# bfloat16/latent-diffusion-speech

Hardware: AMD Instinct MI355X
Metric: mel_frames_per_sec (higher is better)
Workload: dtype f32; 1 GPU; configs[1]: batch=16x512-frame utterances per GPU, 50-step dpm-solver, unet1d denoiser, 80-ch mel; pipeline=sampler, utterances_per_gpu=16, frames=512, nfe=50, method=dpm-solver, parallelism=batch-shard x1

## Files before the change

latent-diffusion-speech_amd/csrc/host_stub_hip.cpp:

```cpp
#include <hip/hip_runtime_api.h>

#include <stdlib.h>
#include <string.h>

extern "C" {
hipError_t hipMalloc(void** p, size_t n) {
    *p = malloc(n ? n : 1);
    return *p ? hipSuccess : hipErrorOutOfMemory;
}
hipError_t hipFree(void* p) {
    free(p);
    return hipSuccess;
}
hipError_t hipMemcpy(void* d, const void* s, size_t n, hipMemcpyKind) {
    memcpy(d, s, n);
    return hipSuccess;
}
hipError_t hipMemcpyAsync(void* d, const void* s, size_t n, hipMemcpyKind, hipStream_t) {
    memcpy(d, s, n);
    return hipSuccess;
}
hipError_t hipMemsetAsync(void* d, int v, size_t n, hipStream_t) {
    memset(d, v, n);
    return hipSuccess;
}
hipError_t hipMemcpy2DAsync(void* d, size_t dpitch, const void* s_, size_t spitch, size_t width, size_t height, hipMemcpyKind, hipStream_t) {
    for (size_t r = 0; r < height; ++r) memcpy((char*)d + r * dpitch, (const char*)s_ + r * spitch, width);
    return hipSuccess;
}
hipError_t hipMemsetD32Async(hipDeviceptr_t d, int v, size_t count, hipStream_t) {
    for (size_t i = 0; i < count; ++i) memcpy((char*)d + 4 * i, &v, 4);
    return hipSuccess;
}
hipError_t hipStreamSynchronize(hipStream_t) { return hipSuccess; }
hipError_t hipGetDevice(int* d) {
    *d = 0;
    return hipSuccess;
}
hipError_t hipGetLastError(void) { return hipSuccess; }
hipError_t hipDeviceGetAttribute(int*, hipDeviceAttribute_t, int) { return hipErrorNotSupported; }
const char* hipGetErrorString(hipError_t) { return "host stub"; }
hipError_t hipFuncSetAttribute(const void*, hipFuncAttribute, int) { return hipSuccess; }
hipError_t hipLaunchKernel(const void*, dim3, dim3, void**, size_t, hipStream_t) { return hipErrorNotSupported; }
hipError_t hipExtLaunchKernel(const void*, dim3, dim3, void**, size_t, hipStream_t, hipEvent_t, hipEvent_t, int) { return hipErrorNotSupported; }
hipError_t hipEventCreate(hipEvent_t*) { return hipErrorNotSupported; }
hipError_t hipEventDestroy(hipEvent_t) { return hipSuccess; }
hipError_t hipEventRecord(hipEvent_t, hipStream_t) { return hipErrorNotSupported; }
hipError_t hipEventSynchronize(hipEvent_t) { return hipErrorNotSupported; }
hipError_t hipEventElapsedTime(float*, hipEvent_t, hipEvent_t) { return hipErrorNotSupported; }
void** __hipRegisterFatBinary(const void*) {
    static void* handle = nullptr;
    return &handle;
}
void __hipRegisterFunction(void**, const void*, char*, const char*, unsigned int, void*, void*, void*, void*, int*) {}
void __hipRegisterVar(void**, void*, char*, const char*, int, size_t, int, int) {}
void __hipUnregisterFatBinary(void**) {}
hipError_t __hipPushCallConfiguration(dim3, dim3, size_t, hipStream_t) { return hipSuccess; }
hipError_t __hipPopCallConfiguration(dim3*, dim3*, size_t*, hipStream_t*) { return hipErrorNotSupported; }
}
```

latent-diffusion-speech_amd/csrc/kernels.h:

```cpp
#pragma once
#include <hip/hip_runtime.h>
#include <stddef.h>
#include <stdint.h>

#include <atomic>
#include <string>

namespace lds {

enum { ACT_NONE = 0, ACT_LRELU = 2 };
enum { EPI_NONE = 0, EPI_GEGLU = 1, EPI_TANH = 2, EPI_GELU = 3, EPI_SWISH = 4, EPI_GLU = 5 };

struct ConvArgs {
    const float* x1; const float* x2;
    int C1, C2;
    int Tsrc;
    int Tin;
    long long xb1, xb2;
    const float* w;
    int Mp, Co, Ci, KT, stride, dil, pad, ups;
    int act_in; float slope;
    const float* bias;
    const float* bias_bc;
    const float* res;
// ... 151 lines not shown
hipError_t launch_w2v_lnpart(const float* x, float2* part, const int* nlen, int B, int C, int T, hipStream_t s);

constexpr int kW2vbertRelStride = 80;
hipError_t launch_w2vbert_fbank(const float* audio, const int* slen, long long L, int Nmax, int Rmax, const double* basis, const float* filtT, int n_mels,
                                int stride, float mel_floor, float* logspec, double2* stat, float* out, int B, hipStream_t s);
hipError_t launch_w2vbert_feats_k4p(const float* feats, float* out, float2* part, const int* vlen, int B, int C, int T, hipStream_t s);
hipError_t launch_w2vbert_relpos(const float* qk, const float* E, float* relp, const int* qlen, int B, int C, int T, int heads, int NR, hipStream_t s);
hipError_t launch_attention_k4p_rel(const float* qk, const float* vt, const float* relp, float* out, int B, int C, int T, int heads, const int* qlens,
                                    const int* klens, int left, int right, hipStream_t s);
hipError_t launch_w2vbert_dwconv(const float* x, const float* wp, const float* gamma, const float* beta, float eps, float* out, const int* vlen,
                                 const int* nlen, int B, int C, int T, int K, hipStream_t s);

enum { IN_PLAIN = 0, IN_SILU = 1, IN_SINUSOID = 2 };
hipError_t launch_small_linear(const float* W, const float* bias, const float* in, int in_stride, int in_mode,
                               const float* freqs, float* out, int out_stride, int out_silu, int M, int K, int B, hipStream_t s);

enum {
    EW_X0 = 1,
    EW_AXPBY = 2,
    EW_DPM2 = 3,
    EW_UNIPC_PRED = 4,
    EW_UNIPC_CORR = 5,
    EW_UNIPC_CORR1 = 6,
    EW_DDPM = 7,
    EW_DDIM = 8,
    EW_PLMS_PRED = 9,
    EW_LIN4 = 10,
    EW_COPY = 11
};
hipError_t launch_ew(int op, float* out, const float* a, const float* b, const float* c, const float* d,
                     float c0, float c1, float c2, float c3, float c4, long long n, hipStream_t s);
hipError_t launch_dpm_step(float* x, const float* eps, float* m0, const float* m1, float sigma, float alpha, int second, float c4, float c5, float c6,
                           float c7, long long n, hipStream_t s);
hipError_t launch_fill(float* p, float v, long long n, hipStream_t s);
hipError_t launch_touch_lines(const float* p, long long bytes, hipStream_t s);
struct FloatList64 { float f[64]; };
hipError_t launch_set_list(float* dst, const float* host, int n, hipStream_t s);
hipError_t launch_transpose(const float* in, float* out, int B, int R, int C, float scale, hipStream_t s);
hipError_t launch_gather_rows(const float* table, const int64_t* idx, int idx_off, float* out, int B, int C,
                              int nrows, hipStream_t s);
hipError_t launch_resample_frames(const float* in, float* out, int B, int Tin, int Tout, int C, float step, hipStream_t s);
hipError_t launch_resample_nearest(const float* in, float* out, int B, int C, int Tin, int Tout, hipStream_t s);


bool prof_attach_events(hipEvent_t* start, hipEvent_t* stop);
int set_error(int code, const char* fmt, ...);

struct ProfScope {
    bool on;
    hipStream_t s;
    int idx = -1;
    bool attached = false;
    ProfScope(hipStream_t st, const char* name, double flops, double bytes, bool attachable = false);
    ~ProfScope();
    void rename(const std::string& n);
};

inline hipError_t ensure_max_dynamic_lds(const void* kern, std::atomic<unsigned long long>& done) {
    int dev = 0;
    hipError_t e = hipGetDevice(&dev);
    if (e != hipSuccess) return e;
    const unsigned long long bit = 1ull << (dev & 63);
    if (done.load(std::memory_order_acquire) & bit) return hipSuccess;
    e = hipFuncSetAttribute(kern, hipFuncAttributeMaxDynamicSharedMemorySize, 160 * 1024);
    if (e == hipSuccess) done.fetch_or(bit, std::memory_order_release);
    return e;
// ... 4 lines not shown
```

latent-diffusion-speech_amd/csrc/misc.hip:

```cpp
#include "kernels.h"
#include "../../include/lds.h"

#include <math.h>

namespace lds {

template <int BT>
__global__ void __launch_bounds__(256) small_linear_kernel(const float* __restrict__ W, const float* __restrict__ bias,
                                                           const float* __restrict__ in, int in_stride, int in_mode,
                                                           const float* __restrict__ freqs, float* __restrict__ out,
                                                           int out_stride, int out_silu, int M, int K, int B) {
    const int lane = threadIdx.x & 63;
    const int m = blockIdx.x * 4 + (threadIdx.x >> 6);
    if (m >= M) return;
    const float* wr = W + (long long)m * K;
    for (int b0 = 0; b0 < B; b0 += BT) {
        float acc[BT];
#pragma unroll
        for (int i = 0; i < BT; ++i) acc[i] = 0.f;
        for (int k = lane * 4; k < K; k += 256) {
            const float4 w4 = *reinterpret_cast<const float4*>(wr + k);
            const float wv[4] = {w4.x, w4.y, w4.z, w4.w};
#pragma unroll
            for (int i = 0; i < BT; ++i) {
// ... 68 lines not shown
            default: r = a[i]; break;
        }
        out[i] = r;
    }
}

hipError_t launch_ew(int op, float* out, const float* a, const float* b, const float* c, const float* d, float c0, float c1,
                     float c2, float c3, float c4, long long n, hipStream_t s) {
    long long blocks = (n + 255) / 256;
    if (blocks > 4096) blocks = 4096;
    ProfScope ps(s, "ew", 0.0, 4.0 * 3.0 * (double)n);
    hipLaunchKernelGGL(ew_kernel, dim3((unsigned)blocks), dim3(256), 0, s, op, out, a, b, c, d, c0, c1, c2, c3, c4, n);
    return hipGetLastError();
}

__global__ void __launch_bounds__(256) dpm_step_kernel(float* __restrict__ x, const float* __restrict__ eps, float* __restrict__ m0, const float* __restrict__ m1,
                                                       float sigma, float alpha, int second, float c4, float c5, float c6, float c7, long long n) {
    for (long long i = (long long)blockIdx.x * 256 + threadIdx.x; i < n; i += (long long)gridDim.x * 256) {
        const float xi = x[i];
        const float bi = (xi - sigma * eps[i]) / alpha;
        m0[i] = bi;
        x[i] = second ? c4 * xi - c5 * bi - c6 * (c7 * (bi - m1[i])) : c4 * xi - c5 * bi;
    }
}
hipError_t launch_dpm_step(float* x, const float* eps, float* m0, const float* m1, float sigma, float alpha, int second, float c4, float c5, float c6,
                           float c7, long long n, hipStream_t s) {
    long long blocks = (n + 255) / 256;
    if (blocks > 4096) blocks = 4096;
    ProfScope ps(s, "ew", 0.0, 4.0 * (second ? 5.0 : 4.0) * (double)n);
    hipLaunchKernelGGL(dpm_step_kernel, dim3((unsigned)blocks), dim3(256), 0, s, x, eps, m0, m1, sigma, alpha, second, c4, c5, c6, c7, n);
    return hipGetLastError();
}

__global__ void __launch_bounds__(256) fill_kernel(float* p, float v, long long n) {
    for (long long i = (long long)blockIdx.x * 256 + threadIdx.x; i < n; i += (long long)gridDim.x * 256) p[i] = v;
}
__global__ void __launch_bounds__(256) touch_lines_kernel(const float* p, long long n_lines, float* sink) {
    const long long i = (long long)blockIdx.x * 256 + threadIdx.x;
    float v = 0.f;
    if (i < n_lines) v = p[i * 16];
    if (v == 1.2345678e-30f && sink) sink[0] = v;
}
hipError_t launch_touch_lines(const float* p, long long bytes, hipStream_t s) {
    const long long n_lines = bytes / 64;
    if (n_lines <= 0) return hipSuccess;
    hipLaunchKernelGGL(touch_lines_kernel, dim3((unsigned)((n_lines + 255) / 256)), dim3(256), 0, s, p, n_lines, (float*)nullptr);
    return hipGetLastError();
}

hipError_t launch_fill(float* p, float v, long long n, hipStream_t s) {
    long long blocks = (n + 255) / 256;
    if (blocks > 4096) blocks = 4096;
    ProfScope ps(s, "fill", 0.0, 4.0 * (double)n);
    hipLaunchKernelGGL(fill_kernel, dim3((unsigned)blocks), dim3(256), 0, s, p, v, n);
    return hipGetLastError();
}

__global__ void __launch_bounds__(64) set_list_kernel(float* __restrict__ dst, FloatList64 v, int n) {
    if ((int)threadIdx.x < n) dst[threadIdx.x] = v.f[threadIdx.x];
}
hipError_t launch_set_list(float* dst, const float* host, int n, hipStream_t s) {
    if (n < 0 || n > 64) return hipErrorInvalidValue;
    FloatList64 v;
    for (int i = 0; i < 64; ++i) v.f[i] = i < n ? host[i] : 0.f;
    hipLaunchKernelGGL(set_list_kernel, dim3(1), dim3(64), 0, s, dst, v, n);
    return hipGetLastError();
// ... 171 lines not shown
```

latent-diffusion-speech_amd/csrc/model.hip:

```cpp
#include "../../include/lds.h"
#include "../../include/lds_test.h"
#include "k4p.h"
#include "k8b3.h"
#include "kernels.h"

#include <math.h>
#include <stdarg.h>
#include <stdio.h>
#include <stdlib.h>
#include <string.h>

#include <algorithm>
#include <atomic>
#include <map>
#include <mutex>
#include <string>
#include <vector>

using namespace lds;

static thread_local char g_err[512] = "";
static int fail(int code, const char* fmt, ...) {
    va_list ap;
    va_start(ap, fmt);
// ... 647 lines not shown
    return LDS_OK;
}

static int dconv_any(int mode, const ConvW& W, const float* x1, int C1, const float* x2, int C2, int Tsrc, const DOpt& o, float* out, int B, hipStream_t st) {
    return mode ? run_dconv_bf3(W, x1, C1, x2, C2, Tsrc, o, out, B, st, 0, mode - 1) : run_dconv(W, x1, C1, x2, C2, Tsrc, o, out, B, st);
}
static hipError_t gn_any(int mode, const float* x1, const float* x2, int C1, int C2, int T, int groups, float eps, const float* gamma, const float* beta,
                         const float* ss, int ss_stride, int ss_off, int silu, const float2* gp1, const float2* gp2, float* y, int B, hipStream_t s, int lvl = 0) {
    return mode ? launch_gn_stream_bf3(x1, x2, C1, C2, T, groups, eps, gamma, beta, ss, ss_stride, ss_off, silu, gp1, gp2, y, B, s, mode - 1, tl_lens, lvl)
                : launch_gn_stream(x1, x2, C1, C2, T, groups, eps, gamma, beta, ss, ss_stride, ss_off, silu, gp1, gp2, y, B, s, tl_lens, lvl);
}
static hipError_t to_act_any(int mode, const float* in, float* out, int B, int C, int T, int Ctot, int c_off, hipStream_t s) {
    return mode ? launch_to_k8b3(in, out, B, C, T, Ctot, c_off, s, mode - 1, tl_lens) : launch_to_k4p(in, out, B, C, T, Ctot, c_off, s, tl_lens);
}

struct ResnetW {
    int cin = 0, cout = 0;
    float *g1 = nullptr, *b1 = nullptr, *g2 = nullptr, *b2 = nullptr;
    ConvW conv1, conv2, sc;
    float* bias_pair = nullptr;
    bool has_sc = false;
    int temb_off = 0;
};
struct TfmW {
    int C = 0;
    float *gn_g = nullptr, *gn_b = nullptr;
    float *qkv_c1[2] = {nullptr, nullptr}, *qkv_c2[2] = {nullptr, nullptr}, *ff1_c1 = nullptr, *ff1_c2 = nullptr;
    ConvW proj_in, qkv[2], o[2], ff1, ff2_out;
    ConvW proj_in_g; float *pi_cg = nullptr, *pi_c2 = nullptr; bool fold = false;
};
struct DownBlk { std::vector<ResnetW> res; std::vector<TfmW> att; bool has_down = false; ConvW down; int ch = 0; };
struct UpBlk { std::vector<ResnetW> res; std::vector<TfmW> att; std::vector<int> skip_ch; bool has_up = false; ConvW up; int ch = 0; };

struct lds_unet {
    lds_unet_cfg cfg;
    Owner own;
    int M = 0, H = 0, G = 8, heads = 8, temb = 0, tproj_dim = 0;
    ConvW conv_in, conv_out;
    ConvW conv_in_x, conv_in_c;
    float *gno_g = nullptr, *gno_b = nullptr;
    float* freqs = nullptr;
    float *t_w1 = nullptr, *t_b1 = nullptr, *t_w2 = nullptr, *t_b2 = nullptr;
    float *tp_w = nullptr, *tp_b = nullptr;
    int tp_M = 0;
    std::vector<DownBlk> down;
    ResnetW mid_r0, mid_r1;
    TfmW mid_t;
    std::vector<UpBlk> up;
    int max_ci = 0;
    int gemm_mode = LDS_GEMM_F32;
    bool split_packed[2] = {false, false};
    int latency_mode = 0;
    std::atomic<int> in_calls{0};
};
struct UnetCallScope {
    lds_unet* u;
    explicit UnetCallScope(lds_unet* u_) : u(u_) { u->in_calls.fetch_add(1, std::memory_order_acq_rel); }
    ~UnetCallScope() { u->in_calls.fetch_sub(1, std::memory_order_acq_rel); }
};

static float* up_vec(Owner& o, const float* p, int64_t n) {
    if (!p) return nullptr;
    return o.upload(std::vector<float>(p, p + n));
}

static bool load_resnet(lds_unet* u, Tensors& T, const std::string& p, int cin, int cout, std::vector<float>& tpw,
                        std::vector<float>& tpb, ResnetW& r) {
    Owner& o = u->own;
    r.cin = cin; r.cout = cout;
    r.g1 = up_vec(o, T.get(p + "norm1.weight", cin), cin);
    r.b1 = up_vec(o, T.get(p + "norm1.bias", cin), cin);
    r.g2 = up_vec(o, T.get(p + "norm2.weight", cout), cout);
    r.b2 = up_vec(o, T.get(p + "norm2.bias", cout), cout);
    const float* w1 = T.get(p + "conv1.weight", (int64_t)cout * cin * 3);
    const float* c1b = T.get(p + "conv1.bias", cout);
    const float* w2 = T.get(p + "conv2.weight", (int64_t)cout * cout * 3);
    const float* c2b = T.get(p + "conv2.bias", cout);
    const float* tw = T.get(p + "time_emb_proj.weight", (int64_t)2 * cout * u->temb);
    const float* tb = T.get(p + "time_emb_proj.bias", 2 * cout);
    if (!r.g1 || !r.b1 || !r.g2 || !r.b2 || !w1 || !c1b || !w2 || !c2b || !tw || !tb) return false;
    if (!pack_conv(o, w1, c1b, cout, cin, 3, r.conv1)) return false;
    if (!pack_conv(o, w2, c2b, cout, cout, 3, r.conv2)) return false;
    r.has_sc = cin != cout;
    if (r.has_sc) {
        const float* ws = T.get(p + "conv_shortcut.weight", (int64_t)cout * cin);
// ... 173 lines not shown
        for (int j = 0; j < L + 1 && ok; ++j) {
            const int sk = skip_ch.back();
            skip_ch.pop_back();
            const int hin = j == 0 ? prev : cout;
            b.skip_ch.push_back(sk);
            ResnetW r;
            ok = load_resnet(u, T, p + "resnets." + std::to_string(j) + ".", hin + sk, cout, tpw, tpb, r);
            b.res.push_back(r);
            if (i != 0 && ok) {
                TfmW t;
                ok = load_tfm(u, T, p + "attentions." + std::to_string(j) + ".", cout, t);
                b.att.push_back(t);
            }
        }
        if (!last && ok) {
            b.has_up = true;
            const float* w = T.get(p + "upsamplers.0.conv.weight", (int64_t)cout * cout * 3);
            const float* bb = T.get(p + "upsamplers.0.conv.bias", cout);
            ok = w && bb && pack_conv(o, w, bb, cout, cout, 3, b.up);
        }
        u->up.push_back(b);
    }
    if (ok) {
        u->gno_g = up_vec(o, T.get("conv_norm_out.weight", boc[0]), boc[0]);
        u->gno_b = up_vec(o, T.get("conv_norm_out.bias", boc[0]), boc[0]);
        const float* w = T.get("conv_out.weight", (int64_t)u->M * boc[0] * 3);
        const float* b = T.get("conv_out.bias", u->M);
        ok = u->gno_g && u->gno_b && w && b && pack_conv(o, w, b, u->M, boc[0], 3, u->conv_out);
    }
    if (ok) {
        u->tp_M = (int)tpb.size();
        u->tp_w = o.upload(tpw);
        u->tp_b = o.upload(tpb);
        ok = u->tp_w && u->tp_b;
    }
    if (cin0 > u->max_ci) u->max_ci = cin0;
    if (!ok) {
        std::string miss = T.missing;
        delete u;
        if (!miss.empty()) return fail(LDS_EMISSING, "weight tensor %s", miss.c_str());
        return fail(LDS_ENOMEM, "device allocation / upload failed while packing weights");
    }
    *out = u;
    return LDS_OK;
}

extern "C" void lds_unet_destroy(lds_unet* u) { delete u; }

static bool unet_pack_split(lds_unet* u, int fmt) {
    Owner& o = u->own;
    bool ok = true;
    auto T1 = [&](ConvW& W) { ok = ok && make_split_twin(o, W, fmt); };
    auto res = [&](ResnetW& r) {
        T1(r.conv1);
        if (r.has_sc) ok = ok && make_split_twin_pair(o, r.conv2, r.sc, fmt);
        else T1(r.conv2);
    };
    auto tfm = [&](TfmW& t) { T1(t.proj_in); if (t.fold) T1(t.proj_in_g); T1(t.qkv[0]); T1(t.qkv[1]); T1(t.o[0]); T1(t.o[1]); T1(t.ff1); T1(t.ff2_out); };
    T1(u->conv_in); T1(u->conv_in_x); T1(u->conv_in_c); T1(u->conv_out);
    for (auto& d : u->down) {
        for (auto& r : d.res) res(r);
        for (auto& t : d.att) tfm(t);
        if (d.has_down) T1(d.down);
    }
    res(u->mid_r0); tfm(u->mid_t); res(u->mid_r1);
    for (auto& b : u->up) {
        for (auto& r : b.res) res(r);
// ... 233 lines not shown
    for (int b = 0; b < B; ++b) {
        if (lens_host[b] < 1 || lens_host[b] > T) return fail(LDS_EINVAL, "length[%d] = %d outside 1 .. %d", b, lens_host[b], T);
        memcpy(&tmp[b], &lens_host[b], sizeof(int));
    }
    HIP_TRY(launch_set_list((float*)dev, tmp, B, st));
    return LDS_OK;
}

static int time_embedding(const lds_unet* u, const float* t, float* e1, float* emb, float* tproj, int n, hipStream_t st) {
    HIP_TRY(launch_small_linear(u->t_w1, u->t_b1, t, 1, IN_SINUSOID, u->freqs, e1, u->temb, 1, u->temb, u->tproj_dim, n, st));
    HIP_TRY(launch_small_linear(u->t_w2, u->t_b2, e1, u->temb, IN_PLAIN, nullptr, emb, u->temb, 1, u->temb, u->temb, n, st));
    HIP_TRY(launch_small_linear(u->tp_w, u->tp_b, emb, u->temb, IN_PLAIN, nullptr, tproj, u->tp_M, 0, u->tp_M, u->temb, n, st));
    return LDS_OK;
}

static int unet_stage_cond(lds_unet* u, const float* cond, void* ws, size_t ws_bytes, int B, int T, hipStream_t st, const int* lens_host = nullptr) {
    Arena A(ws, ws_bytes);
    UnetWs w;
    plan_ws(u, A, B, T, w);
    if (!A.ok) return fail(LDS_ENOMEM, "unet workspace too small: need %zu bytes, got %zu", A.used, ws_bytes);
    if (lens_host) LDS_TRY(upload_lens(u, lens_host, B, T, w.lens_dev, st));
    LensScope lsc(lens_host ? w.lens_dev : nullptr);
    TileBatchScope tbs(u->latency_mode ? B : 0, w.kpart, w.kcount);
    if (u->latency_mode) HIP_TRY(launch_fill((float*)w.kcount, 0.f, kClusterCounters, st));
    const int bf3 = u->gemm_mode;
    HIP_TRY(to_act_any(bf3, cond, w.ck, B, u->H, T, u->H, 0, st));
    DOpt o;
    o.pad = 1;
    return dconv_any(bf3, u->conv_in_c, w.ck, u->H, nullptr, 0, T, o, w.cinc, B, st);
}

static int unet_forward_impl(lds_unet* u, const float* x, const float* cond, const float* t, float* eps, void* ws, size_t ws_bytes,
                             int B, int T, hipStream_t st, bool uniform_t = false, const float* tproj_pre = nullptr,
                             bool cond_staged = false, const int* lens_host = nullptr) {
    UnetCallScope in_call(u);
    Arena A(ws, ws_bytes);
    UnetWs w;
    plan_ws(u, A, B, T, w);
    if (!A.ok) return fail(LDS_ENOMEM, "unet workspace too small: need %zu bytes, got %zu", A.used, ws_bytes);
    if (lens_host && !cond_staged) LDS_TRY(upload_lens(u, lens_host, B, T, w.lens_dev, st));
    LensScope lsc(lens_host ? w.lens_dev : nullptr);
    TileBatchScope tbs(u->latency_mode ? B : 0, w.kpart, w.kcount);
    if (u->latency_mode && !cond_staged) HIP_TRY(launch_fill((float*)w.kcount, 0.f, kClusterCounters, st));
    const int nb = u->cfg.n_blocks;
    const int bf3 = u->gemm_mode;
    const int Bt = uniform_t ? 1 : B;
    w.ss_stride = (uniform_t || tproj_pre) ? 0 : u->tp_M;
    if (tproj_pre) {
        w.tproj = const_cast<float*>(tproj_pre);
    } else {
        LDS_TRY(time_embedding(u, t, w.e1, w.emb, w.tproj, Bt, st));
    }
    const int cin = u->M + u->H;
    size_t si = 0;
    if (cond_staged) {
        HIP_TRY(to_act_any(bf3, x, w.xk, B, u->M, T, u->M, 0, st));
        DOpt o;
        o.pad = 1; o.res = w.cinc; o.gnpart_out = w.gp(w.skips[si]);
        LDS_TRY(dconv_any(bf3, u->conv_in_x, w.xk, u->M, nullptr, 0, T, o, w.skips[si], B, st));
    } else {
        HIP_TRY(to_act_any(bf3, x, w.xin, B, u->M, T, cin, 0, st));
        HIP_TRY(to_act_any(bf3, cond, w.xin, B, u->H, T, cin, u->M, st));
        DOpt o;
        o.pad = 1; o.gnpart_out = w.gp(w.skips[si]);
        LDS_TRY(dconv_any(bf3, u->conv_in, w.xin, cin, nullptr, 0, T, o, w.skips[si], B, st));
    }
    const bool tr = g_trace_on.load(std::memory_order_relaxed) != 0;
    auto stage = [&](const char* fmt, int i, int j) { if (tr) { char nm[48]; snprintf(nm, sizeof(nm), fmt, i, j); tl_trace_stage = nm; } };
    stage("conv_in", 0, 0);
    TRACE_ACT("out", w.skips[si], u->conv_in.Co, T);
    const float* cur = w.skips[si++];
    int Tl = T, lvl = 0;
    std::vector<int> skipT{T};
    for (int i = 0; i < nb; ++i) {
        const DownBlk& d = u->down[i];
        for (size_t j = 0; j < d.res.size(); ++j) {
            float* dst = w.skips[si];
            const bool att = !d.att.empty();
            stage("down%d.res%d", i, (int)j);
            LDS_TRY(run_resnet(u, d.res[j], w, cur, d.res[j].cin, nullptr, 0, Tl, att ? w.r : dst, B, st, lvl));
            stage("down%d.tfm%d", i, (int)j);
            if (att) LDS_TRY(run_tfm(u, d.att[j], w, w.r, Tl, dst, B, st, lvl));
            cur = dst;
            ++si;
            skipT.push_back(Tl);
        }
        if (d.has_down) {
            DOpt o;
            o.lvl_in = lvl; o.lvl_out = lvl + 1;
// ... 48 lines not shown
                HIP_TRY(bf3 ? launch_resample_k8b3(cur, w.upt, B, b.ch, Tl, Tn, st, bf3 - 1, tl_lens, lvl, lvl - 1) : launch_resample_k4p(cur, w.upt, B, b.ch, Tl, Tn, st, tl_lens, lvl, lvl - 1));
                LDS_TRY(dconv_any(bf3, b.up, w.upt, b.ch, nullptr, 0, Tn, o, dst, B, st));
            }
            Tl = Tn;
            --lvl;
            stage("up%d.upsample", i, 0);
            TRACE_ACT("out", dst, b.ch, Tl);
            cur = dst;
            ci ^= 1;
        }
    }
    const int c0 = u->cfg.block_out_channels[0];
    HIP_TRY(gn_any(bf3, cur, nullptr, c0, 0, Tl, u->G, 1e-5f, u->gno_g, u->gno_b, nullptr, 0, 0, 1, w.gp(cur), nullptr, w.gno, B, st, 0));
    stage("out", 0, 0);
    TRACE_ACT("gn", w.gno, c0, Tl);
    DOpt o;
    o.pad = 1; o.out_plain = 1;
    LDS_TRY(dconv_any(bf3, u->conv_out, w.gno, c0, nullptr, 0, Tl, o, eps, B, st));
    TRACE("eps", eps, sizeof(float) * (size_t)B * u->M * Tl);
    return LDS_OK;
}

extern "C" int lds_unet_forward(lds_unet* u, const float* x, const float* cond, const float* t, float* eps, void* ws, size_t ws_bytes,
                                int B, int T, void* stream) {
    if (!u || !x || !cond || !t || !eps || !ws || B <= 0 || T <= 0) return fail(LDS_EINVAL, "bad argument");
    return unet_forward_impl(u, x, cond, t, eps, ws, ws_bytes, B, T, (hipStream_t)stream);
}
extern "C" int lds_unet_forward_ragged(lds_unet* u, const float* x, const float* cond, const float* t, const int32_t* lengths, float* eps, void* ws,
                                       size_t ws_bytes, int B, int T, void* stream) {
    if (!u || !x || !cond || !t || !lengths || !eps || !ws || B <= 0 || T <= 0) return fail(LDS_EINVAL, "bad argument");
    return unet_forward_impl(u, x, cond, t, eps, ws, ws_bytes, B, T, (hipStream_t)stream, false, nullptr, false, lengths);
}

constexpr int kTimePre = 64;
struct SampWs { float *tvec, *eps, *m0, *m1, *m2, *xt, *xp, *tp_t, *tp_e1, *tp_emb, *tp_proj; size_t unet_off; };

static void plan_samp(const lds_unet* u, Arena& A, int B, int T, SampWs& s) {
    const size_t n = (size_t)B * u->M * T;
    s.tvec = A.f(B);
    s.eps = A.f(n); s.m0 = A.f(n); s.m1 = A.f(n); s.m2 = A.f(n); s.xt = A.f(n); s.xp = A.f(n);
    s.tp_t = A.f(kTimePre); s.tp_e1 = A.f((size_t)kTimePre * u->temb); s.tp_emb = A.f((size_t)kTimePre * u->temb);
    s.tp_proj = A.f((size_t)kTimePre * u->tp_M);
    s.unet_off = A.used;
}

extern "C" int lds_sampler_workspace_bytes(const lds_unet* u, int B, int T, size_t* out) {
    if (!u || !out || B <= 0 || T <= 0) return fail(LDS_EINVAL, "bad argument");
    Arena A(nullptr, 0);
    SampWs s;
    plan_samp(u, A, B, T, s);
    size_t un = 0;
    LDS_TRY(lds_unet_workspace_bytes(u, B, T, &un));
    *out = A.used + un;
    return LDS_OK;
}

static int sampler_run_impl(lds_unet* u, int method, int n_rows, const float* table, const float* cond, float* x, const float* noise, void* ws, size_t ws_bytes,
                            int B, int T, void* stream, const int* lens);
extern "C" int lds_sampler_run(lds_unet* u, int method, int n_rows, const float* table, const float* cond, float* x,
                               const float* noise, void* ws, size_t ws_bytes, int B, int T, void* stream) {
    return sampler_run_impl(u, method, n_rows, table, cond, x, noise, ws, ws_bytes, B, T, stream, nullptr);
}
extern "C" int lds_sampler_run_ragged(lds_unet* u, int method, int n_rows, const float* table, const float* cond, float* x, const float* noise,
                                      const int32_t* lengths, void* ws, size_t ws_bytes, int B, int T, void* stream) {
    if (!lengths) return fail(LDS_EINVAL, "bad argument");
    return sampler_run_impl(u, method, n_rows, table, cond, x, noise, ws, ws_bytes, B, T, stream, lengths);
}
static int sampler_run_impl(lds_unet* u, int method, int n_rows, const float* table, const float* cond, float* x, const float* noise, void* ws, size_t ws_bytes,
                            int B, int T, void* stream, const int* lens) {
    if (!u || !table || !cond || !x || !ws || n_rows <= 0 || B <= 0 || T <= 0) return fail(LDS_EINVAL, "bad argument");
    UnetCallScope in_call(u);
    hipStream_t st = (hipStream_t)stream;
    ProfChain chain;
    Arena A(ws, ws_bytes);
    SampWs s;
    plan_samp(u, A, B, T, s);
    if (!A.ok || A.used > ws_bytes) return fail(LDS_ENOMEM, "sampler workspace too small");
    void* uws = (char*)ws + s.unet_off;
    const size_t uws_bytes = ws_bytes - s.unet_off;
    const long long n = (long long)B * u->M * T;
    const int S = LDS_TABLE_STRIDE;
    std::vector<float> tlist;
    for (int i = 0; i < n_rows; ++i) tlist.push_back(table[(size_t)i * S]);
    if (method == LDS_METHOD_PLMS) tlist.push_back(table[1]);
    const bool pre = (int)tlist.size() <= kTimePre;
    if (pre) {
        HIP_TRY(launch_set_list(s.tp_t, tlist.data(), (int)tlist.size(), st));
        LDS_TRY(time_embedding(u, s.tp_t, s.tp_e1, s.tp_emb, s.tp_proj, (int)tlist.size(), st));
    }
    LDS_TRY(unet_stage_cond(u, cond, uws, uws_bytes, B, T, st, lens));
    auto model = [&](const float* xin, float t_in) -> int {
        if (pre) {
            for (size_t i = 0; i < tlist.size(); ++i)
                if (tlist[i] == t_in)
                    return unet_forward_impl(u, xin, cond, nullptr, s.eps, uws, uws_bytes, B, T, st, true, s.tp_proj + i * u->tp_M, true, lens);
        }
        HIP_TRY(launch_fill(s.tvec, t_in, B, st));
        return unet_forward_impl(u, xin, cond, s.tvec, s.eps, uws, uws_bytes, B, T, st, true, nullptr, true, lens);
    };
    float *m0 = s.m0, *m1 = s.m1, *m2 = s.m2;
    if (method == LDS_METHOD_DPM_SOLVER_PP) {
        for (int i = 0; i < n_rows; ++i) {
            const float* r = table + (size_t)i * S;
            LDS_TRY(model(x, r[0]));
            float* tmp = m1; m1 = m0; m0 = tmp;
            HIP_TRY(launch_dpm_step(x, s.eps, m0, m1, r[1], r[2], r[3] < 1.5f ? 0 : 1, r[4], r[5], r[6], r[7], n, st));
        }
    } else if (method == LDS_METHOD_UNIPC) {
        LDS_TRY(model(x, table[0]));
        HIP_TRY(launch_ew(EW_X0, m0, x, s.eps, nullptr, nullptr, table[1], table[2], 0, 0, 0, n, st));
        for (int i = 1; i < n_rows; ++i) {
            const float* r = table + (size_t)i * S;
            const bool o2 = r[3] > 1.5f, corr = r[11] > 0.5f;
            HIP_TRY(launch_ew(EW_AXPBY, s.xt, x, m0, nullptr, nullptr, r[4], r[5], 0, 0, 0, n, st));
            const float* xpred = s.xt;
            if (o2) {
                HIP_TRY(launch_ew(EW_UNIPC_PRED, s.xp, s.xt, m0, m1, nullptr, r[6], r[8], r[7], 0, 0, n, st));
                xpred = s.xp;
            }
            if (corr) {
                LDS_TRY(model(xpred, r[0]));
                HIP_TRY(launch_ew(EW_X0, m2, xpred, s.eps, nullptr, nullptr, r[1], r[2], 0, 0, 0, n, st));
                if (o2) HIP_TRY(launch_ew(EW_UNIPC_CORR, x, s.xt, m0, m2, m1, r[6], r[9], r[7], r[10], 0, n, st));
                else HIP_TRY(launch_ew(EW_UNIPC_CORR1, x, s.xt, m0, m2, nullptr, r[6], 0, 0, r[10], 0, n, st));
                float* tmp = m1; m1 = m0; m0 = m2; m2 = tmp;
            } else {
                HIP_TRY(launch_ew(EW_COPY, x, xpred, nullptr, nullptr, nullptr, 0, 0, 0, 0, 0, n, st));
            }
        }
    } else if (method == LDS_METHOD_DDPM) {
        if (!noise) return fail(LDS_EINVAL, "DDPM needs per-step noise");
        for (int i = 0; i < n_rows; ++i) {
            const float* r = table + (size_t)i * S;
            LDS_TRY(model(x, r[0]));
            HIP_TRY(launch_ew(EW_DDPM, x, x, s.eps, noise + (size_t)i * n, nullptr, r[1], r[2], r[3], r[4], r[5], n, st));
        }
    } else if (method == LDS_METHOD_DDIM) {
        for (int i = 0; i < n_rows; ++i) {
            const float* r = table + (size_t)i * S;
// ... 2211 lines not shown
    TmpDev tmp;
    DownW d;
    d.w = own.upload(std::vector<float>(w, w + (size_t)Co * Ci * K));
    if (b) d.bias = own.upload(std::vector<float>(b, b + Co));
    if (!d.w || (b && !d.bias)) return fail(LDS_ENOMEM, "upload failed");
    d.Co = Co; d.Ci = Ci; d.K = K; d.stride = stride; d.pad = pad;
    int* vl[2] = {nullptr, nullptr};
    for (int i = 0; i < 2 && lengths_in; ++i) {
        float t4[64];
        memcpy(t4, src[i], sizeof(int) * B);
        vl[i] = (int*)tmp.f(64);
        if (!vl[i]) return fail(LDS_ENOMEM, "alloc");
        HIP_TRY(launch_set_list((float*)vl[i], t4, B, st));
    }
    LDS_TRY(run_down(d, x, T, slope, out, B, st, tile, vl[0], vl[1]));
    if (cfg_out && cfg_cap) snprintf(cfg_out, cfg_cap, "%s", conv_down_last_config());
    HIP_TRY(hipStreamSynchronize(st));
    return LDS_OK;
}
extern "C" int lds_test_conv_down(const float* x, const float* w, const float* b, int Ci, int Co, int K, int stride, int T, int B, float slope,
                                  int tile, float* out, char* cfg_out, size_t cfg_cap, void* stream) {
    return conv_down_test_impl(x, w, b, Ci, Co, K, stride, T, B, slope, nullptr, nullptr, tile, out, cfg_out, cfg_cap, stream);
}
extern "C" int lds_test_conv_down_ragged(const float* x, const float* w, const float* b, int Ci, int Co, int K, int stride, int T, int B, float slope,
                                         const int32_t* lengths_in, const int32_t* lengths_out, int tile, float* out, char* cfg_out, size_t cfg_cap,
                                         void* stream) {
    if (!lengths_in || !lengths_out || B < 1 || B > 64) return fail(LDS_EINVAL, "bad argument: lengths_in / lengths_out null or B %d outside 1 .. 64", B);
    return conv_down_test_impl(x, w, b, Ci, Co, K, stride, T, B, slope, lengths_in, lengths_out, tile, out, cfg_out, cfg_cap, stream);
}
extern "C" int lds_debug_set_gn_fold(int on) {
    g_gn_fold.store(on ? 1 : 0);
    return LDS_OK;
}
extern "C" int lds_debug_set_split_rule(int rule) {
    conv_bf3_set_debug_rule(rule);
    return LDS_OK;
}

static int test_upload_lens(TmpDev& tmp, const int32_t* host, int B, int*& dev, hipStream_t st) {
    dev = nullptr;
    if (!host) return LDS_OK;
    if (B < 1 || B > 64) return fail(LDS_EINVAL, "per-utterance lengths: 1 .. 64 batch elements (got %d)", B);
    dev = (int*)tmp.f(64);
    if (!dev) return fail(LDS_ENOMEM, "alloc");
    float t4[64];
    memcpy(t4, host, sizeof(int) * B);
    HIP_TRY(launch_set_list((float*)dev, t4, B, st));
    return LDS_OK;
}
struct TestActs {
    int fmt, B; hipStream_t st;
    size_t floats(int C, int T) const { return fmt < 0 ? (size_t)B * C * (T + 2) : (size_t)B * split_floats(fmt, C, T); }
    hipError_t to(const float* src, float* dst, int C, int T) const { return fmt < 0 ? launch_to_k4p(src, dst, B, C, T, C, 0, st) : launch_to_k8b3(src, dst, B, C, T, C, 0, st, fmt); }
    hipError_t from(const float* src, float* dst, int C, int T) const { return fmt < 0 ? launch_from_k4p(src, dst, B, C, T, st) : launch_from_k8b3(src, dst, B, C, T, st, fmt); }
};

extern "C" int lds_test_dconv_pair(const float* h, const float* x1, const float* x2, const float* w3, const float* b3, const float* w1, const float* b1, int B,
                                   int Cm, int C1, int C2, int Co, int T, const int32_t* lengths, int lvl, int tile_batch, int fmt, float* out, float* gnpart,
                                   char* cfg_out, size_t cfg_cap, void* stream) {
    hipStream_t st = (hipStream_t)stream;
    if (!h || !x1 || (C2 > 0) != (x2 != nullptr) || !w3 || !b3 || !w1 || !b1 || !out || !gnpart || B < 1 || T < 1 || Cm < 8 || C1 < 8 || C2 < 0 || (Cm & 7) || (C1 & 7) ||
        (C2 & 7) || Co < 32 || Co % 32 || lvl < 0 || tile_batch < 0 || (fmt != -1 && fmt != FMT_BF16X3 && fmt != FMT_F16X2))
        return fail(LDS_EINVAL, "bad argument");
    const bool f32 = fmt < 0;
    Owner own;
    TmpDev tmp;
// ... 305 lines not shown
```

latent-diffusion-speech_amd/lds/native.py:

```python
import ctypes as C
import os

import numpy as np

_HERE = os.path.dirname(os.path.abspath(__file__))
LIB_PATH = os.path.join(_HERE, "liblds.so")
_lib = None

METHODS = {"dpm-solver": 1, "unipc": 2, "ddpm": 3, "ddim": 4, "pndm": 5}
TABLE_STRIDE = 16


class UNetCfg(C.Structure):
    _fields_ = [("out_dims", C.c_int), ("n_hidden", C.c_int), ("n_layers", C.c_int), ("n_heads", C.c_int),
                ("norm_groups", C.c_int), ("n_blocks", C.c_int), ("block_out_channels", C.c_int * 8)]


class VocoderCfg(C.Structure):
    _fields_ = [("inter_channels", C.c_int), ("upsample_initial_channel", C.c_int), ("n_ups", C.c_int),
                ("upsample_rates", C.c_int * 8), ("upsample_kernel_sizes", C.c_int * 8), ("resblock", C.c_int),
                ("n_kernels", C.c_int), ("resblock_kernel_sizes", C.c_int * 4), ("n_dil", C.c_int),
                ("resblock_dilation_sizes", (C.c_int * 4) * 4)]


# ... 124 lines not shown
lds_volume_mask                  i:ppqifp
lds_resample_frames_ragged       i:ppppiiiip
lds_overlap_assemble             i:pqppipqpqp
lds_prof_enable                  i:i
lds_prof_summary                 i:pz
lds_unet_set_gemm_mode           i:pi
lds_unet_get_gemm_mode           i:p
lds_unet_set_latency_mode        i:pi
lds_unet_get_latency_mode        i:p
"""
_TEST = """
lds_test_conv                    i:ppip
lds_test_dconv                   i:pppip
lds_bench_dconv                  i:ppiippzp
lds_test_gn_apply                i:ppiiiifpppipip
lds_bench_gn_stream              i:iiiiipp
lds_test_gn_chain_k4p            i:pppppfiippiiiiip
lds_test_ln_chain_k4p            i:pppppfppiiiip
lds_test_attention_k4p           i:ppiiiip
lds_test_conv_transpose          i:ppppiiiiiiifp
lds_test_voc_step                i:pppppiiiiipfppip
lds_test_dconv_bf3               i:pppiip
lds_bench_dconv_bf3              i:ppiiippzp
lds_test_k8b3_roundtrip          i:ppiiip
lds_test_gn_apply_bf3            i:ppiiiifpppipip
lds_test_dconv_split             i:pppiiip
lds_bench_dconv_split            i:ppiiiippzp
lds_test_split_roundtrip         i:ppiiiip
lds_test_gn_apply_split          i:ppiiiifpppipiip
lds_debug_set_split_rule         i:i
lds_test_attention_f16math       i:ppiiiip
lds_test_attention_latency       i:ppiiiiip
lds_debug_set_gn_fold            i:i
lds_debug_set_voc_pair           i:i
lds_debug_set_touch_weights      i:i
lds_test_voc_pair                i:pppppiiiipfppip
lds_test_gn_fold_k4p             i:pppppfippppiiiiiiip
lds_bench_dconv_alt              i:ppiipipp
lds_debug_fill_u32               i:pzup
lds_debug_trace                  i:i
lds_debug_trace_count            i:
lds_debug_trace_get              i:ipzpp
lds_debug_unet_plan              i:piipz
lds_test_gn_fold_split           i:pppppfippppiiiiiiiiip
lds_test_cluster_join            i:ppppiiiiiiippppzp
lds_test_lm_sample               i:piiiifffppipp
lds_test_conv_down               i:pppiiiiiifippzp
lds_test_conv_down_ragged        i:pppiiiiiifppippzp
lds_test_lm_beam_step            i:piiiiiifiippppppppppppppppp
lds_test_dconv_pair              i:pppppppiiiiiipiiipppzp
lds_test_dconv_ex                i:pppipzp
lds_test_dma_magic_div           i:uup
lds_test_dma_tile_order          i:iiiip
lds_test_tap_k4p                 i:pz
lds_test_voc_ups                 i:pppiiiiiipppppzp
lds_test_w2v_conv0               i:ppppppfpiiqp
lds_test_w2v_ln_act              i:ppppfppiiip
lds_test_w2vbert_fbank           i:pppiqp
lds_test_w2vbert_attention       i:pppppiiiiiip
lds_test_w2vbert_dwconv          i:ppppfpppiiiip
lds_test_stft_dft                i:pppiiiippiqp
"""
SIGNATURES = dict(ln.split() for ln in (_PUBLIC + _TEST).splitlines() if ln)
EXPORTS = [ln.split()[0] for ln in _PUBLIC.splitlines() if ln]
TEST_EXPORTS = [ln.split()[0] for ln in _TEST.splitlines() if ln]

# ... 1050 lines not shown
```

Before: 24350 mel-frames/s.

## Fuse DPM-solver update with k4p staging and cache time-embedding projections

The DPM-solver step kernel now also writes the updated latent directly into the UNet's packed k4p input buffer, with padded time edges. The next UNet call can therefore skip its separate to_act_any layout conversion of x. Separately, the per-model time-embedding projections are cached, keyed on the timestep list, and reused across sampler calls. Events and a reader count guard the shared cache buffer. This adds cross-stream event synchronisation and a persistent buffer, and the fused path only applies in f32 GEMM mode without ragged lengths.

Measured after the change: 24430 mel-frames/s (median of 6 runs). Within noise of the previous version (+0.3%).

```diff
diff --git a/latent-diffusion-speech_amd/csrc/host_stub_hip.cpp b/latent-diffusion-speech_amd/csrc/host_stub_hip.cpp
--- a/latent-diffusion-speech_amd/csrc/host_stub_hip.cpp
+++ b/latent-diffusion-speech_amd/csrc/host_stub_hip.cpp
@@ -44,9 +44,12 @@
 hipError_t hipLaunchKernel(const void*, dim3, dim3, void**, size_t, hipStream_t) { return hipErrorNotSupported; }
 hipError_t hipExtLaunchKernel(const void*, dim3, dim3, void**, size_t, hipStream_t, hipEvent_t, hipEvent_t, int) { return hipErrorNotSupported; }
 hipError_t hipEventCreate(hipEvent_t*) { return hipErrorNotSupported; }
+hipError_t hipEventCreateWithFlags(hipEvent_t*, unsigned) { return hipErrorNotSupported; }
 hipError_t hipEventDestroy(hipEvent_t) { return hipSuccess; }
 hipError_t hipEventRecord(hipEvent_t, hipStream_t) { return hipErrorNotSupported; }
 hipError_t hipEventSynchronize(hipEvent_t) { return hipErrorNotSupported; }
+hipError_t hipEventQuery(hipEvent_t) { return hipErrorNotSupported; }
+hipError_t hipStreamWaitEvent(hipStream_t, hipEvent_t, unsigned) { return hipErrorNotSupported; }
 hipError_t hipEventElapsedTime(float*, hipEvent_t, hipEvent_t) { return hipErrorNotSupported; }
 void** __hipRegisterFatBinary(const void*) {
     static void* handle = nullptr;
diff --git a/latent-diffusion-speech_amd/csrc/kernels.h b/latent-diffusion-speech_amd/csrc/kernels.h
--- a/latent-diffusion-speech_amd/csrc/kernels.h
+++ b/latent-diffusion-speech_amd/csrc/kernels.h
@@ -207,6 +207,8 @@
                      float c0, float c1, float c2, float c3, float c4, long long n, hipStream_t s);
 hipError_t launch_dpm_step(float* x, const float* eps, float* m0, const float* m1, float sigma, float alpha, int second, float c4, float c5, float c6,
                            float c7, long long n, hipStream_t s);
+hipError_t launch_dpm_step_k4p(float* x, const float* eps, float* m0, const float* m1, float* xk, int B, int M, int T, float sigma, float alpha, int second,
+                               float c4, float c5, float c6, float c7, hipStream_t s);
 hipError_t launch_fill(float* p, float v, long long n, hipStream_t s);
 hipError_t launch_touch_lines(const float* p, long long bytes, hipStream_t s);
 struct FloatList64 { float f[64]; };
diff --git a/latent-diffusion-speech_amd/csrc/misc.hip b/latent-diffusion-speech_amd/csrc/misc.hip
--- a/latent-diffusion-speech_amd/csrc/misc.hip
+++ b/latent-diffusion-speech_amd/csrc/misc.hip
@@ -124,6 +124,39 @@
     return hipGetLastError();
 }
 
+typedef float dpm_f32x4 __attribute__((ext_vector_type(4)));
+__global__ void __launch_bounds__(256) dpm_step_k4p_kernel(float* __restrict__ x, const float* __restrict__ eps, float* __restrict__ m0, const float* __restrict__ m1,
+                                                           float* __restrict__ xk, int M, int T, float sigma, float alpha, int second, float c4, float c5,
+                                                           float c6, float c7) {
+    const int q = blockIdx.x, b = blockIdx.y, Tp = T + 2;
+    const int idx = blockIdx.z * 256 + threadIdx.x;
+    if (idx >= 2 * Tp) return;
+    const int hh = idx / Tp, e = idx - hh * Tp, t = e - 1;
+    dpm_f32x4 v = {0.f, 0.f, 0.f, 0.f};
+    if (t >= 0 && t < T) {
+#pragma unroll
+        for (int j = 0; j < 4; ++j) {
+            const long long i = ((long long)b * M + q * 8 + 2 * j + hh) * T + t;
+            const float xi = x[i];
+            const float bi = (xi - sigma * eps[i]) / alpha;
+            m0[i] = bi;
+            const float xn = second ? c4 * xi - c5 * bi - c6 * (c7 * (bi - m1[i])) : c4 * xi - c5 * bi;
+            x[i] = xn;
+            v[j] = xn;
+        }
+    }
+    *reinterpret_cast<dpm_f32x4*>(xk + ((((long long)b * (M >> 3) + q) * 2) * Tp + idx) * 4) = v;
+}
+hipError_t launch_dpm_step_k4p(float* x, const float* eps, float* m0, const float* m1, float* xk, int B, int M, int T, float sigma, float alpha, int second,
+                               float c4, float c5, float c6, float c7, hipStream_t s) {
+    if (!xk || B <= 0 || M <= 0 || (M & 7) || T <= 0 || B > 65535) return hipErrorInvalidValue;
+    const double n = (double)B * M * T;
+    ProfScope ps(s, "ew", 0.0, 4.0 * (second ? 6.0 : 5.0) * n);
+    hipLaunchKernelGGL(dpm_step_k4p_kernel, dim3(M / 8, B, (2 * (T + 2) + 255) / 256), dim3(256), 0, s, x, eps, m0, m1, xk, M, T, sigma, alpha, second, c4, c5,
+                       c6, c7);
+    return hipGetLastError();
+}
+
 __global__ void __launch_bounds__(256) fill_kernel(float* p, float v, long long n) {
     for (long long i = (long long)blockIdx.x * 256 + threadIdx.x; i < n; i += (long long)gridDim.x * 256) p[i] = v;
 }
diff --git a/latent-diffusion-speech_amd/csrc/model.hip b/latent-diffusion-speech_amd/csrc/model.hip
--- a/latent-diffusion-speech_amd/csrc/model.hip
+++ b/latent-diffusion-speech_amd/csrc/model.hip
@@ -703,6 +703,22 @@
 struct DownBlk { std::vector<ResnetW> res; std::vector<TfmW> att; bool has_down = false; ConvW down; int ch = 0; };
 struct UpBlk { std::vector<ResnetW> res; std::vector<TfmW> att; std::vector<int> skip_ch; bool has_up = false; ConvW up; int ch = 0; };
 
+constexpr int kTimePre = 64;
+struct TimeCache {
+    std::mutex mu;
+    float* buf = nullptr;
+    std::vector<float> tl;
+    hipEvent_t filled = nullptr;
+    int readers = 0;
+    std::vector<hipEvent_t> done;
+    ~TimeCache() {
+        if (filled) (void)hipEventDestroy(filled);
+        for (hipEvent_t e : done) (void)hipEventDestroy(e);
+    }
+};
+static std::atomic<int> g_dpm_k4p{1};
+static std::atomic<int> g_time_cache{1};
+
 struct lds_unet {
     lds_unet_cfg cfg;
     Owner own;
@@ -722,6 +738,7 @@
     int gemm_mode = LDS_GEMM_F32;
     bool split_packed[2] = {false, false};
     int latency_mode = 0;
+    TimeCache tc;
     std::atomic<int> in_calls{0};
 };
 struct UnetCallScope {
@@ -961,7 +978,8 @@
         u->tp_M = (int)tpb.size();
         u->tp_w = o.upload(tpw);
         u->tp_b = o.upload(tpb);
-        ok = u->tp_w && u->tp_b;
+        u->tc.buf = o.upload(std::vector<float>((size_t)kTimePre * u->tp_M, 0.f));
+        ok = u->tp_w && u->tp_b && u->tc.buf;
     }
     if (cin0 > u->max_ci) u->max_ci = cin0;
     if (!ok) {
@@ -1261,7 +1279,7 @@
 
 static int unet_forward_impl(lds_unet* u, const float* x, const float* cond, const float* t, float* eps, void* ws, size_t ws_bytes,
                              int B, int T, hipStream_t st, bool uniform_t = false, const float* tproj_pre = nullptr,
-                             bool cond_staged = false, const int* lens_host = nullptr) {
+                             bool cond_staged = false, const int* lens_host = nullptr, bool x_staged = false) {
     UnetCallScope in_call(u);
     Arena A(ws, ws_bytes);
     UnetWs w;
@@ -1283,7 +1301,7 @@
     const int cin = u->M + u->H;
     size_t si = 0;
     if (cond_staged) {
-        HIP_TRY(to_act_any(bf3, x, w.xk, B, u->M, T, u->M, 0, st));
+        if (!x_staged) HIP_TRY(to_act_any(bf3, x, w.xk, B, u->M, T, u->M, 0, st));
         DOpt o;
         o.pad = 1; o.res = w.cinc; o.gnpart_out = w.gp(w.skips[si]);
         LDS_TRY(dconv_any(bf3, u->conv_in_x, w.xk, u->M, nullptr, 0, T, o, w.skips[si], B, st));
@@ -1398,7 +1416,6 @@
     return unet_forward_impl(u, x, cond, t, eps, ws, ws_bytes, B, T, (hipStream_t)stream, false, nullptr, false, lengths);
 }
 
-constexpr int kTimePre = 64;
 struct SampWs { float *tvec, *eps, *m0, *m1, *m2, *xt, *xp, *tp_t, *tp_e1, *tp_emb, *tp_proj; size_t unet_off; };
 
 static void plan_samp(const lds_unet* u, Arena& A, int B, int T, SampWs& s) {
@@ -1421,6 +1438,24 @@
     return LDS_OK;
 }
 
+struct TimeCacheReader {
+    lds_unet* u;
+    hipStream_t st;
+    bool reading = false;
+    TimeCacheReader(lds_unet* u_, hipStream_t st_) : u(u_), st(st_) {}
+    ~TimeCacheReader() {
+        if (!reading) return;
+        TimeCache& tc = u->tc;
+        std::lock_guard<std::mutex> lk(tc.mu);
+        hipEvent_t ev = nullptr;
+        for (hipEvent_t e : tc.done)
+            if (hipEventQuery(e) == hipSuccess) { ev = e; break; }
+        (void)hipGetLastError();
+        if (!ev && hipEventCreateWithFlags(&ev, hipEventDisableTiming) == hipSuccess) tc.done.push_back(ev);
+        if (!ev || hipEventRecord(ev, st) != hipSuccess) { (void)hipStreamSynchronize(st); }
+        --tc.readers;
+    }
+};
 static int sampler_run_impl(lds_unet* u, int method, int n_rows, const float* table, const float* cond, float* x, const float* noise, void* ws, size_t ws_bytes,
                             int B, int T, void* stream, const int* lens);
 extern "C" int lds_sampler_run(lds_unet* u, int method, int n_rows, const float* table, const float* cond, float* x,
@@ -1450,27 +1485,64 @@
     for (int i = 0; i < n_rows; ++i) tlist.push_back(table[(size_t)i * S]);
     if (method == LDS_METHOD_PLMS) tlist.push_back(table[1]);
     const bool pre = (int)tlist.size() <= kTimePre;
+    const float* tproj = s.tp_proj;
+    TimeCacheReader tcr(u, st);
     if (pre) {
-        HIP_TRY(launch_set_list(s.tp_t, tlist.data(), (int)tlist.size(), st));
-        LDS_TRY(time_embedding(u, s.tp_t, s.tp_e1, s.tp_emb, s.tp_proj, (int)tlist.size(), st));
+        TimeCache& tc = u->tc;
+        std::unique_lock<std::mutex> lk(tc.mu);
+        const bool use = g_time_cache.load(std::memory_order_relaxed) != 0;
+        float* dst = s.tp_proj;
+        bool fill = true;
+        if (use && !tc.tl.empty() && tc.tl == tlist) {
+            if (hipEventQuery(tc.filled) != hipSuccess) HIP_TRY(hipStreamWaitEvent(st, tc.filled, 0));
+            (void)hipGetLastError();
+            fill = false;
+            tproj = tc.buf;
+            tcr.reading = true; ++tc.readers;
+        } else if (use && tc.readers == 0) {
+            for (hipEvent_t e : tc.done) HIP_TRY(hipStreamWaitEvent(st, e, 0));
+            if (!tc.filled) HIP_TRY(hipEventCreateWithFlags(&tc.filled, hipEventDisableTiming));
+            tc.tl.clear();
+            dst = tc.buf;
+        }
+        if (fill) {
+            HIP_TRY(launch_set_list(s.tp_t, tlist.data(), (int)tlist.size(), st));
+            LDS_TRY(time_embedding(u, s.tp_t, s.tp_e1, s.tp_emb, dst, (int)tlist.size(), st));
+            if (dst == tc.buf) {
+                HIP_TRY(hipEventRecord(tc.filled, st));
+                tc.tl = tlist;
+                tproj = tc.buf;
+                tcr.reading = true; ++tc.readers;
+            }
+        }
     }
     LDS_TRY(unet_stage_cond(u, cond, uws, uws_bytes, B, T, st, lens));
-    auto model = [&](const float* xin, float t_in) -> int {
+    auto model = [&](const float* xin, float t_in, bool x_staged = false) -> int {
         if (pre) {
             for (size_t i = 0; i < tlist.size(); ++i)
                 if (tlist[i] == t_in)
-                    return unet_forward_impl(u, xin, cond, nullptr, s.eps, uws, uws_bytes, B, T, st, true, s.tp_proj + i * u->tp_M, true, lens);
+                    return unet_forward_impl(u, xin, cond, nullptr, s.eps, uws, uws_bytes, B, T, st, true, tproj + i * u->tp_M, true, lens, x_staged);
         }
         HIP_TRY(launch_fill(s.tvec, t_in, B, st));
-        return unet_forward_impl(u, xin, cond, s.tvec, s.eps, uws, uws_bytes, B, T, st, true, nullptr, true, lens);
+        return unet_forward_impl(u, xin, cond, s.tvec, s.eps, uws, uws_bytes, B, T, st, true, nullptr, true, lens, x_staged);
     };
     float *m0 = s.m0, *m1 = s.m1, *m2 = s.m2;
     if (method == LDS_METHOD_DPM_SOLVER_PP) {
+        float* xk = nullptr;
+        if (g_dpm_k4p.load(std::memory_order_relaxed) && u->gemm_mode == LDS_GEMM_F32 && !lens && u->M % 8 == 0) {
+            Arena UA(uws, uws_bytes);
+            UnetWs uw;
+            plan_ws(u, UA, B, T, uw);
+            if (UA.ok) xk = uw.xk;
+        }
+        bool staged = false;
         for (int i = 0; i < n_rows; ++i) {
             const float* r = table + (size_t)i * S;
-            LDS_TRY(model(x, r[0]));
+            LDS_TRY(model(x, r[0], staged));
             float* tmp = m1; m1 = m0; m0 = tmp;
-            HIP_TRY(launch_dpm_step(x, s.eps, m0, m1, r[1], r[2], r[3] < 1.5f ? 0 : 1, r[4], r[5], r[6], r[7], n, st));
+            staged = xk && i + 1 < n_rows;
+            if (staged) HIP_TRY(launch_dpm_step_k4p(x, s.eps, m0, m1, xk, B, u->M, T, r[1], r[2], r[3] < 1.5f ? 0 : 1, r[4], r[5], r[6], r[7], st));
+            else HIP_TRY(launch_dpm_step(x, s.eps, m0, m1, r[1], r[2], r[3] < 1.5f ? 0 : 1, r[4], r[5], r[6], r[7], n, st));
         }
     } else if (method == LDS_METHOD_UNIPC) {
         LDS_TRY(model(x, table[0]));
@@ -3748,6 +3820,14 @@
     g_gn_fold.store(on ? 1 : 0);
     return LDS_OK;
 }
+extern "C" int lds_debug_set_dpm_k4p(int on) {
+    g_dpm_k4p.store(on ? 1 : 0);
+    return LDS_OK;
+}
+extern "C" int lds_debug_set_time_cache(int on) {
+    g_time_cache.store(on ? 1 : 0);
+    return LDS_OK;
+}
 extern "C" int lds_debug_set_split_rule(int rule) {
     conv_bf3_set_debug_rule(rule);
     return LDS_OK;
diff --git a/latent-diffusion-speech_amd/lds/native.py b/latent-diffusion-speech_amd/lds/native.py
--- a/latent-diffusion-speech_amd/lds/native.py
+++ b/latent-diffusion-speech_amd/lds/native.py
@@ -180,6 +180,8 @@
 lds_test_attention_f16math       i:ppiiiip
 lds_test_attention_latency       i:ppiiiiip
 lds_debug_set_gn_fold            i:i
+lds_debug_set_time_cache         i:i
+lds_debug_set_dpm_k4p            i:i
 lds_debug_set_voc_pair           i:i
 lds_debug_set_touch_weights      i:i
 lds_test_voc_pair                i:pppppiiiipfppip
```
